# ShigemichiMatsuzaki/MSPL

Measured on AMD Instinct MI355X. Metric: images/sec pseudo-label gen, ESPDNet-UE s=2.0 480x360(->288x480) bs=16, higher is better.
Workload: dtype f32; 1 GPU; BASELINE configs[1]: ESPDNet-UE s=2.0 C=13 single-source pseudo-label gen (forward + pred+0.5aux argmax + KL uncertainty + histogram), bs=16/GPU, 16x3x288x480 fp32, hipGraph replay, 3 launches in flight per GPU, 2 consecutive batches of 16 per launch; per_gpu_batch=16, batches_in_flight=3, batches_per_launch=2, classes=13

## Files before the change

include/mspl_hip.h:

```cpp
#ifndef MSPL_HIP_H
#define MSPL_HIP_H

#include <stddef.h>
#include <stdint.h>

#ifdef __cplusplus
extern "C" {
#endif

typedef enum {
    MSPL_OK = 0,
    MSPL_ERR_BAD_SHAPE = -1,
    MSPL_ERR_UNSUPPORTED = -2,
    MSPL_ERR_NULL_POINTER = -3,
    MSPL_ERR_HIP = -4
} mspl_status;

typedef struct {
    const float* scale;
    const float* shift;
    const float* alpha;
    const float* pre_add;
    const float* residual;
    const float* reinf_r;
// ... 12 lines not shown

const char* mspl_version(void);
int mspl_abi_version(void);
size_t mspl_last_error(char* buf, size_t cap);

int mspl_eesp_dw_hff_fwd(const float* x, const float* w, const int32_t dil[4], int32_t stride,
                         int32_t N, int32_t n, int32_t H, int32_t W,
                         const mspl_epilogue_t* ep, float* out, void* stream);

int mspl_conv1x1_fwd(const float* x, const float* w, int32_t N, int32_t Cin, int32_t Cout,
                     int32_t groups, int32_t HW, const mspl_epilogue_t* ep, float* out, void* stream);

int mspl_conv3x3_fwd(const float* x, const float* w, int32_t N, int32_t Cin, int32_t Cout,
                     int32_t groups, int32_t H, int32_t W, int32_t stride, int32_t shuffle_groups,
                     const mspl_epilogue_t* ep, float* out, void* stream);

int mspl_eesp_proj_dw_hff_fits(int32_t N, int32_t Cin, int32_t n, int32_t groups, int32_t H, int32_t W, const int32_t dil[4],
                               uint32_t launch_flags);
int mspl_eesp_proj_dw_hff_fwd(const float* x, const float* wp, const float* pscale, const float* pshift, const float* palpha,
                              const float* w, const int32_t dil[4], int32_t N, int32_t Cin, int32_t n, int32_t groups,
                              int32_t H, int32_t W, const mspl_epilogue_t* ep, float* out, void* stream);

int mspl_eesp_dw_exp_fits(int32_t N, int32_t n, int32_t H, int32_t W, const int32_t dil[4], uint32_t launch_flags);
int64_t mspl_eesp_dw_exp_pack_floats(int32_t n);
int mspl_eesp_dw_exp_pack(const float* w4, const float* bscale, const float* bshift, const float* balpha, const float* wexp,
                          int32_t n, int32_t H, int32_t W, const int32_t dil[4], float* packed, void* stream);
int mspl_eesp_dw_exp_fwd(const float* r, const float* packed, const int32_t dil[4], int32_t N, int32_t n, int32_t H, int32_t W,
                         const mspl_epilogue_t* ep, float* out, void* stream);
int64_t mspl_eesp_dw_exp_next_pack_floats(int32_t n);
int mspl_eesp_dw_exp_next_pack(const float* w1, int32_t n, float* next_packed, void* stream);
int mspl_eesp_dw_exp_next_fwd(const float* r, const float* packed, const int32_t dil[4], int32_t N, int32_t n, int32_t H, int32_t W,
                              const mspl_epilogue_t* ep, float* out, const float* next_packed, const float* nscale,
                              const float* nshift, const float* nalpha, float* rnext, void* stream);

int mspl_avgpool3x3s2_fwd(const float* x, int32_t N, int32_t C, int32_t H, int32_t W,
                          const mspl_epilogue_t* ep, float* out, void* stream);

int mspl_bilinear_fwd(const float* x, int32_t N, int32_t C, int32_t Hi, int32_t Wi, int32_t Ho,
                      int32_t Wo, int32_t align_corners, const mspl_epilogue_t* ep, float* out, void* stream);

int mspl_adaptive_avgpool_fwd(const float* x, int32_t N, int32_t C, int32_t Hi, int32_t Wi,
                              int32_t Ho, int32_t Wo, const mspl_epilogue_t* ep, float* out,
                              void* stream);

int mspl_pointwise_fwd(const float* x, int32_t N, int32_t C, int32_t HW, const mspl_epilogue_t* ep,
                       float* out, void* stream);

int mspl_gap_gate_fwd(const float* x, const float* w, int32_t N, int32_t Cin, int32_t Cout,
                      int32_t HW, float* mean_ws, float* gate, void* stream);

int mspl_fusion_gate_fwd(const float* z, const float* rgb, const float* depth, int64_t count, float* out, void* stream);
int mspl_fusion_gate_bwd(const float* z, const float* rgb, const float* depth, const float* gy, int64_t count,
                         float* gz, float* grgb, float* gdepth, void* stream);

int mspl_avgpool3x3s2_psum_blocks(int32_t H, int32_t W);
int mspl_avgpool3x3s2_psum_fwd(const float* x, int32_t N, int32_t C, int32_t H, int32_t W, const mspl_epilogue_t* ep, float* out,
                               float* psum, void* stream);
int mspl_gate_from_sums_fwd(const float* psum, const float* w, int32_t N, int32_t Cin, int32_t Cout, int32_t nblk, int32_t HW,
                            float* gate, void* stream);

int64_t mspl_pyr_down_prep_lds_bytes(int32_t N, int32_t P, int32_t h, int32_t w, int32_t nb, const int32_t* hs,
                                     const int32_t* ws);
int mspl_pyr_down_prep_fwd(const float* x, int32_t N, int32_t P, int32_t h, int32_t w, int32_t nb, const int32_t* hs,
                           const int32_t* ws, const float* const* stage_w, float* const* out, void* stream);
int mspl_pyr_down_prep_train_fwd(const float* x, int32_t N, int32_t P, int32_t h, int32_t w, int32_t nb, const int32_t* hs,
                                 const int32_t* ws, const float* const* stage_w, float* const* out, float* const* pooled,
// ... 206 lines not shown
```

mspl_amd/_native.py:

```python
import ctypes
import os

import torch

_HERE = os.path.dirname(os.path.abspath(__file__))
LIB_PATH = os.environ.get('MSPL_HIP_LIB') or os.path.join(_HERE, 'lib', 'libmspl_hip.so')

c_f32p = ctypes.c_void_p
c_i32 = ctypes.c_int32
c_i64 = ctypes.c_int64


class Epilogue(ctypes.Structure):
    _fields_ = [('scale', ctypes.c_void_p), ('shift', ctypes.c_void_p), ('alpha', ctypes.c_void_p),
                ('pre_add', ctypes.c_void_p), ('residual', ctypes.c_void_p), ('reinf_r', ctypes.c_void_p),
                ('reinf_w', ctypes.c_void_p), ('gate', ctypes.c_void_p),
                ('out_ctot', c_i32), ('out_coff', c_i32), ('raw_out', ctypes.c_void_p),
                ('struct_size', ctypes.c_uint32), ('flags', ctypes.c_uint32)]


ABI_VERSION = 3
LAUNCH_THROUGHPUT = 1
LAUNCH_K2_STREAM_OFF = 2
LAUNCH_K2_STREAM_FORCE = 4


_EP = ctypes.POINTER(Epilogue)

SIGNATURES = {
    'mspl_eesp_dw_hff_fwd': [c_f32p, c_f32p, ctypes.POINTER(c_i32), c_i32, c_i32, c_i32, c_i32, c_i32, _EP,
                             c_f32p, ctypes.c_void_p],
    'mspl_eesp_proj_dw_hff_fits': [c_i32] * 6 + [ctypes.POINTER(c_i32), ctypes.c_uint32],
    'mspl_eesp_proj_dw_hff_fwd': [c_f32p] * 6 + [ctypes.POINTER(c_i32)] + [c_i32] * 6 + [_EP, c_f32p, ctypes.c_void_p],
    'mspl_eesp_dw_exp_fits': [c_i32] * 4 + [ctypes.POINTER(c_i32), ctypes.c_uint32],
    'mspl_eesp_dw_exp_pack_floats': [c_i32],
    'mspl_eesp_dw_exp_pack': [c_f32p] * 5 + [c_i32] * 3 + [ctypes.POINTER(c_i32), c_f32p, ctypes.c_void_p],
    'mspl_eesp_dw_exp_fwd': [c_f32p, c_f32p, ctypes.POINTER(c_i32)] + [c_i32] * 4 + [_EP, c_f32p, ctypes.c_void_p],
    'mspl_eesp_dw_exp_next_pack_floats': [c_i32],
    'mspl_eesp_dw_exp_next_pack': [c_f32p, c_i32, c_f32p, ctypes.c_void_p],
    'mspl_eesp_dw_exp_next_fwd': [c_f32p, c_f32p, ctypes.POINTER(c_i32)] + [c_i32] * 4 + [_EP, c_f32p] + [c_f32p] * 5 + [ctypes.c_void_p],
    'mspl_conv1x1_fwd': [c_f32p, c_f32p, c_i32, c_i32, c_i32, c_i32, c_i32, _EP, c_f32p, ctypes.c_void_p],
    'mspl_conv3x3_fwd': [c_f32p, c_f32p, c_i32, c_i32, c_i32, c_i32, c_i32, c_i32, c_i32, c_i32, _EP, c_f32p,
                         ctypes.c_void_p],
    'mspl_avgpool3x3s2_fwd': [c_f32p, c_i32, c_i32, c_i32, c_i32, _EP, c_f32p, ctypes.c_void_p],
    'mspl_bilinear_fwd': [c_f32p, c_i32, c_i32, c_i32, c_i32, c_i32, c_i32, c_i32, _EP, c_f32p, ctypes.c_void_p],
    'mspl_adaptive_avgpool_fwd': [c_f32p, c_i32, c_i32, c_i32, c_i32, c_i32, c_i32, _EP, c_f32p, ctypes.c_void_p],
    'mspl_avgpool3x3s2_psum_fwd': [c_f32p, c_i32, c_i32, c_i32, c_i32, _EP, c_f32p, c_f32p, ctypes.c_void_p],
    'mspl_avgpool3x3s2_psum_blocks': [c_i32, c_i32],
    'mspl_gate_from_sums_fwd': [c_f32p, c_f32p, c_i32, c_i32, c_i32, c_i32, c_i32, c_f32p, ctypes.c_void_p],
    'mspl_pointwise_fwd': [c_f32p, c_i32, c_i32, c_i32, _EP, c_f32p, ctypes.c_void_p],
    'mspl_gap_gate_fwd': [c_f32p, c_f32p, c_i32, c_i32, c_i32, c_i32, c_f32p, c_f32p, ctypes.c_void_p],
    'mspl_fusion_gate_fwd': [c_f32p, c_f32p, c_f32p, c_i64, c_f32p, ctypes.c_void_p],
    'mspl_fusion_gate_bwd': [c_f32p, c_f32p, c_f32p, c_f32p, c_i64, c_f32p, c_f32p, c_f32p, ctypes.c_void_p],
    'mspl_pyrpool_fused_fwd': [c_f32p, c_i32, c_i32, c_i32, c_i32, c_i32, ctypes.POINTER(c_i32), ctypes.POINTER(c_i32),
                               ctypes.POINTER(ctypes.c_void_p), ctypes.POINTER(ctypes.c_void_p), c_f32p, c_f32p, c_f32p,
                               c_f32p, _EP, c_f32p, ctypes.c_void_p],
    'mspl_pyrpool_fused_train_fwd': [c_f32p, c_i32, c_i32, c_i32, c_i32, c_i32, ctypes.POINTER(c_i32), ctypes.POINTER(c_i32),
                                     ctypes.POINTER(ctypes.c_void_p), ctypes.POINTER(ctypes.c_void_p), c_f32p, c_f32p, c_f32p,
                                     c_f32p, _EP, c_f32p, c_f32p, ctypes.c_void_p],
    'mspl_pyrpool_fused_train_fits': [c_i32] * 5 + [ctypes.POINTER(c_i32), ctypes.POINTER(c_i32)],
    'mspl_pyrpool_merge_bwd': [c_f32p] * 3 + [c_i32] * 5 + [c_f32p] * 19 + [ctypes.c_void_p],
    'mspl_pyrpool_branch_bwd_fits': [c_i32] * 5 + [ctypes.POINTER(c_i32), ctypes.POINTER(c_i32)],
    'mspl_pyrpool_branch_bwd': [c_f32p] + [c_i32] * 5 + [ctypes.POINTER(c_i32), ctypes.POINTER(c_i32)] +
                               [ctypes.POINTER(ctypes.c_void_p)] * 3 + [c_f32p, c_f32p, c_f32p, ctypes.c_void_p],
    'mspl_label_epilogue_fwd': [c_f32p, c_f32p, c_i32, c_i32, c_i32, c_i32, c_i32, c_i32, c_i32, c_i32,
                                ctypes.c_void_p, ctypes.c_void_p, c_f32p, c_f32p, c_f32p, c_f32p, ctypes.c_void_p],
    'mspl_label_epilogue_hist_fwd': [c_f32p, c_f32p, c_i32, c_i32, c_i32, c_i32, c_i32, c_i32, c_i32, c_i32,
                                     ctypes.c_void_p, ctypes.c_void_p, c_f32p, ctypes.c_void_p, c_i32, ctypes.c_void_p, c_i64,
                                     ctypes.c_void_p],
    'mspl_label_epilogue_hist_workspace_bytes': [c_i32, c_i32, c_i32],
    'mspl_label_epilogue_hist_fits': [c_i32] * 8,
    'mspl_conv_bwd_data': [c_f32p, c_f32p] + [c_i32] * 10 + [c_f32p, ctypes.c_void_p],
    'mspl_conv_bwd_weight': [c_f32p, c_f32p] + [c_i32] * 10 + [c_f32p, ctypes.c_void_p],
# ... 65 lines not shown
    'mspl_eesp_bwd_fused': [c_f32p] * 4 + [ctypes.POINTER(c_i32)] + [c_f32p] * 5 + [c_i32] * 4 + [c_f32p, ctypes.POINTER(ctypes.c_void_p)] +
                           [c_f32p] * 12 + [ctypes.c_void_p],
    'mspl_eesp_dw_bwd': [c_f32p, c_f32p, c_f32p, ctypes.POINTER(c_i32), c_i32, c_i32, c_i32, c_i32, c_i32, c_f32p,
                         ctypes.POINTER(ctypes.c_void_p), ctypes.c_void_p],
    'mspl_png_writer_create': [c_i32, c_i32],
    'mspl_png_writer_submit': [ctypes.c_void_p, ctypes.c_void_p, c_i32, c_i32, c_i32, ctypes.POINTER(ctypes.c_char_p), ctypes.c_void_p],
    'mspl_png_writer_poll': [ctypes.c_void_p, c_i64, c_i32],
    'mspl_png_writer_destroy': [ctypes.c_void_p],
    'mspl_abi_version': [],
    'mspl_sum_n': [ctypes.POINTER(ctypes.c_void_p), c_i32, c_i64, c_f32p, ctypes.c_void_p],
    'mspl_sum_n_planes': [ctypes.POINTER(ctypes.c_void_p), c_i32, c_f32p, ctypes.c_float, c_i32, c_i32, c_f32p, ctypes.c_void_p],
    'mspl_transpose_weights': [ctypes.c_void_p, ctypes.c_void_p, c_i32, ctypes.c_void_p],
    'mspl_adam_step': [c_f32p, c_f32p, c_f32p, c_f32p, c_i64] + [ctypes.c_float] * 5 + [c_i32, ctypes.c_void_p],
    'mspl_merge_labels_fwd': [ctypes.POINTER(ctypes.c_void_p), c_i32, c_i64, c_i32, c_i32, c_i32, ctypes.c_void_p,
                              ctypes.c_void_p, ctypes.c_void_p],
}


def _load():
    if not os.path.isfile(LIB_PATH):
        raise ImportError(
            'mspl_amd: %s not found. Build it with `python -c "import __graft_entry__ as g; g.build()"` or '
            '`make -C mspl_amd/csrc` (hipcc --offload-arch=gfx950). There is no CPU fallback.' % LIB_PATH)
    lib = ctypes.CDLL(LIB_PATH)
    for name, argtypes in SIGNATURES.items():
        fn = getattr(lib, name)
        fn.argtypes = argtypes
        fn.restype = ctypes.c_int
    lib.mspl_pyr_down_prep_lds_bytes.restype = ctypes.c_int64
    lib.mspl_nid_workspace_floats.restype = ctypes.c_int64
    lib.mspl_eesp_dw_exp_pack_floats.restype = ctypes.c_int64
    lib.mspl_bn_fused_workspace_bytes.restype = ctypes.c_int64
    lib.mspl_eesp_dw_exp_next_pack_floats.restype = ctypes.c_int64
    lib.mspl_label_epilogue_hist_workspace_bytes.restype = ctypes.c_int64
    lib.mspl_png_writer_create.restype = ctypes.c_void_p
    lib.mspl_png_writer_submit.restype = ctypes.c_int64
    lib.mspl_version.restype = ctypes.c_char_p
    if lib.mspl_abi_version() != ABI_VERSION:
        raise ImportError('mspl_amd: %s has ABI revision %d, this package binds revision %d: rebuild the library (make -C mspl_amd/csrc)'
                          % (LIB_PATH, lib.mspl_abi_version(), ABI_VERSION))
    lib.mspl_last_error.argtypes = [ctypes.c_char_p, ctypes.c_size_t]
    lib.mspl_last_error.restype = ctypes.c_size_t
    return lib


lib = _load()


def last_error():
    buf = ctypes.create_string_buffer(512)
    lib.mspl_last_error(buf, 512)
    return buf.value.decode()


def check(status):
    if status != 0:
        raise RuntimeError('mspl_hip (%d): %s' % (status, last_error()))


def version():
    return lib.mspl_version().decode()
```

mspl_amd/layers.py:

```python
import math
import os
import weakref

import torch
from torch import nn

from . import autograd as ag
from . import ops
from .ops import Epi

config_inp_reinf = 3
PYR_SCALES = (2.0, 1.5, 1.0, 0.5, 0.1)


_PARAM_EPOCH = [0]


def bump_param_epoch():
    _PARAM_EPOCH[0] += 1


def _key(tensors):
    return (_PARAM_EPOCH[0],) + tuple((t.data_ptr(), t._version) for t in tensors)

# ... 101 lines not shown
    cur.wait_stream(_side_stream(idx, outs[0].device, cur))
    for t in outs:
        t.record_stream(cur)


def _training_path():
    return torch.is_grad_enabled()


def _conv_train(x, conv):
    if conv.kernel_size[0] == 3 and conv.dilation[0] != 1:
        raise RuntimeError('mspl_amd: dilated 3x3 convolutions only occur inside EESP (fused branch op)')
    return ag.conv(x, conv.weight, conv.stride[0], conv.groups)


def _bn_act(z, bn, alpha=None, pre_add=None, residual=None):
    if bn.training:
        if pre_add is not None:
            z, pre_add = z + pre_add, None
        if _FUSED_BN_TRAIN:
            return ag.bn_train_prelu(z, bn, alpha, residual)
        scale, shift = ag.bn_batch_stats(z, bn)
    else:
        scale, shift = train_fold(bn)
        return ag.bn_prelu(z, bn, scale, shift, alpha, pre_add=pre_add, residual=residual)
    return ag.affine_prelu(z, scale, shift, alpha, pre_add=pre_add, residual=residual)


_FUSED_TRAIN_FWD = os.environ.get('MSPL_TRAIN_FUSED_FWD', '1') != '0'
_EESP_DW_BN = os.environ.get('MSPL_EESP_DW_BN', '1') != '0'
_CONV_SKIP = os.environ.get('MSPL_CONV_SKIP', '1') != '0'
_FUSED_BN_TRAIN = os.environ.get('MSPL_FUSED_BN_TRAIN', '1') != '0'
_FUSED_DW_EXP = os.environ.get('MSPL_EESP_EXP', '1') != '0'
_FUSED_NEXT_PROJ = os.environ.get('MSPL_EESP_NEXT', '1') != '0'
_FUSED_EESP_TRAIN = os.environ.get('MSPL_FUSED_EESP_TRAIN', '1') != '0'
_FUSED_PYR_TRAIN = os.environ.get('MSPL_FUSED_PYR_TRAIN', '1') != '0'


def _conv_bn_act(x, conv, bn, alpha=None, pre_add=None, residual=None):
    if bn.training or not _FUSED_TRAIN_FWD:
        return _bn_act(_conv_train(x, conv), bn, alpha, pre_add, residual)
    if conv.kernel_size[0] == 3 and conv.dilation[0] != 1:
        raise RuntimeError('mspl_amd: dilated 3x3 convolutions only occur inside EESP (fused branch op)')
    scale, shift = train_fold(bn)
    return ag.conv_bn_prelu(x, conv.weight, conv.stride[0], conv.groups, bn, scale, shift, alpha, pre_add, residual)


def train_fold(bn):
    def build():
        scale = bn.weight * ag.frozen_bn_inv(bn)
        return scale, torch.addcmul(bn.bias, bn.running_mean, scale, value=-1.0)
    return cached(bn, 'tfold', [bn.weight, bn.bias, bn.running_mean, bn.running_var], build)


def prefold_frozen_bn(model):
    bns = [m for m in model.modules() if isinstance(m, nn.BatchNorm2d) and not m.training]
    if not bns:
        return
    with torch.no_grad():
        invs = [ag.frozen_bn_inv(m) for m in bns]
        scales = torch._foreach_mul([m.weight for m in bns], invs)
        shifts = torch._foreach_addcmul([m.bias for m in bns], [m.running_mean for m in bns], scales, value=-1.0)
    for m, sc, sh in zip(bns, scales, shifts):
        store = m.__dict__.setdefault('_mspl_cache', {})
        store['tfold'] = (_key([m.weight, m.bias, m.running_mean, m.running_var]), (sc, sh))

# ... 128 lines not shown

class EESP(nn.Module):
    def __init__(self, nIn, nOut, stride=1, k=4, r_lim=7, down_method='esp'):
        super().__init__()
        self.stride = stride
        n = int(nOut / k)
        n1 = nOut - (k - 1) * n
        assert down_method in ['avg', 'esp'], 'One of these is suppported (avg or esp)'
        assert n == n1, "n(={}) and n1(={}) should be equal for Depth-wise Convolution ".format(n, n1)
        if k != 4:
            raise NotImplementedError('mspl_amd: the fused EESP kernel is built for k=4 branches')
        self.proj_1x1 = CBR(nIn, n, 1, stride=1, groups=k)
        self.dilations = eesp_dilations(r_lim, k)
        self.spp_dw = nn.ModuleList(CDilated(n, n, kSize=3, stride=stride, groups=n, d=d) for d in self.dilations)
        self.conv_1x1_exp = CB(nOut, nOut, 1, 1, groups=k)
        self.br_after_cat = BR(nOut)
        self.module_act = nn.PReLU(nOut)
        self.downAvg = True if down_method == 'avg' else False
        self.k = k

    def _dw_weights(self):
        ws = [m.conv.weight for m in self.spp_dw]
        return cached(self, 'w4', ws, lambda: torch.stack([w.reshape(-1, 3, 3) for w in ws]).contiguous())

    def _dw_exp_packed(self, H, W):
        br, exp = self.br_after_cat, self.conv_1x1_exp
        deps = [m.conv.weight for m in self.spp_dw] + [br.bn.weight, br.bn.bias, br.bn.running_mean, br.bn.running_var,
                                                      br.act.weight, exp.conv.weight]

        def build():
            bs, bb = bn_fold(br.bn)
            return ops.eesp_dw_exp_pack(self._dw_weights(), bs, bb, br.act.weight, exp.conv.weight, H, W, self.dilations)
        return cached(self, 'dwexp%dx%d' % (H, W), deps, build)

    def reduce_transform(self, input):
        scale, shift = bn_fold(self.br_after_cat.bn)
        pj = self.proj_1x1
        if ops.eesp_proj_dw_hff_fits(input.shape, pj.conv.out_channels, pj.conv.groups, self.dilations, self.stride):
            ps, pb = bn_fold(pj.bn)
            return ops.eesp_proj_dw_hff(input, pj.conv.weight, ps, pb, pj.act.weight, self._dw_weights(), self.dilations,
                                        pj.conv.groups, Epi(scale, shift, self.br_after_cat.act.weight))
        o1 = pj(input)
        return ops.eesp_dw_hff(o1, self._dw_weights(), self.dilations, self.stride,
                               Epi(scale, shift, self.br_after_cat.act.weight))

    def _forward_train(self, input):
        pj, br, exp = self.proj_1x1, self.br_after_cat, self.conv_1x1_exp
        if _FUSED_EESP_TRAIN and not (pj.bn.training or br.bn.training or exp.bn.training):
            def fold(bn):
                scale, shift = train_fold(bn)
                return {'scale': scale, 'shift': shift, 'mean': bn.running_mean, 'inv': ag.frozen_bn_inv(bn)}
            strided_avg = self.stride == 2 and self.downAvg
            residual = (not strided_avg) and self.stride == 1 and exp.conv.out_channels == input.shape[1]
            cfg = {'stride': self.stride, 'dil': tuple(self.dilations), 'groups': pj.conv.groups, 'residual': residual}
            ws = [m.conv.weight for m in self.spp_dw]
            return ag.EESPFn.apply(input, cfg, fold(pj.bn), fold(br.bn), fold(exp.bn), pj.conv.weight, pj.bn.weight, pj.bn.bias,
                                   pj.act.weight, ws[0], ws[1], ws[2], ws[3], br.bn.weight, br.bn.bias, br.act.weight,
                                   exp.conv.weight, exp.bn.weight, exp.bn.bias, None if strided_avg else self.module_act.weight)
        has_res = self.stride == 1 and exp.conv.out_channels == input.shape[1] and not (self.stride == 2 and self.downAvg)
        skip = input
        if has_res and pj.bn.training and _CONV_SKIP and input.requires_grad:
            z1, skip = ag.conv_skip(input, pj.conv.weight, pj.conv.groups)
            o1 = _bn_act(z1, pj.bn, pj.act.weight)
        else:
            o1 = self.proj_1x1(input)
        if br.bn.training and _EESP_DW_BN and o1.requires_grad:
# ... 105 lines not shown
                rw = (cb.conv.weight.reshape(self.nout, config_inp_reinf) * rs[:, None]).contiguous()
                shift = shift + rb
            return scale.contiguous(), shift.contiguous(), rw
        return cached(self, 'epi%d' % int(with_reinf), deps, build)

    def _forward_train(self, input, input2, alias=None):
        avg_out = ag.avgpool(input)
        eesp_out = self.eesp(input if alias is None else alias)
        reinf = None
        if input2 is not None:
            with torch.no_grad():
                pyr = input2 if isinstance(input2, ImagePyramid) else ImagePyramid(input2)
                img = pyr.at_height(avg_out.shape[2])
            if img.shape[3] != avg_out.shape[3]:
                raise RuntimeError('The size of tensor a (%d) must match the size of tensor b (%d) at non-singleton '
                                   'dimension 3' % (avg_out.shape[3], img.shape[3]))
            reinf = self.inp_reinf(img)
        return ag.down_tail(avg_out, eesp_out, self.act.weight, reinf)

    def forward(self, input, input2=None, _alias=None):
        if _training_path():
            return self._forward_train(input, input2, _alias)
        N, _, H, W = input.shape
        Ho, Wo = (H - 1) // 2 + 1, (W - 1) // 2 + 1
        out = torch.empty((N, self.nout, Ho, Wo), device=input.device, dtype=torch.float32)
        r = None
        if input2 is not None:
            pyr = input2 if isinstance(input2, ImagePyramid) else ImagePyramid(input2)
            with fork(0, (pyr.levels[0],)):
                r = self.inp_reinf[0](pyr.at_height(Ho))
            if r.shape[3] != Wo:
                raise RuntimeError('The size of tensor a (%d) must match the size of tensor b (%d) at non-singleton '
                                   'dimension 3' % (Wo, r.shape[3]))
        cat = self.eesp.reduce_transform(input)
        join(0, (r,))
        scale, shift, rw = self._epilogue_vectors(r is not None)
        ep = Epi(scale, shift, self.act.weight, reinf_r=r, reinf_w=rw)
        _, sums = ops.avgpool3x3s2(input, ep, out=(out, 0), plane_sums=True)
        _remember_plane_sums(input, sums)
        ops.conv1x1(cat, self.eesp.conv_1x1_exp.conv.weight, self.eesp.k, ep, out=(out, self.nin))
        return out


_PLANE_SUMS = weakref.WeakKeyDictionary()


class _TensorKey(object):
    __slots__ = ('__weakref__',)


def _remember_plane_sums(t, sums):
    key = getattr(t, '_mspl_key', None)
    if key is None:
        key = _TensorKey()
        t._mspl_key = key
    _PLANE_SUMS[key] = (t.data_ptr(), t._version, sums)


def _recall_plane_sums(t):
    key = getattr(t, '_mspl_key', None)
    hit = _PLANE_SUMS.get(key) if key is not None else None
    if hit is None or hit[0] != t.data_ptr() or hit[1] != t._version:
        return None
    return hit[2]


class EfficientPyrPool(nn.Module):
    def __init__(self, in_planes, proj_planes, out_planes, scales=[2.0, 1.5, 1.0, 0.5, 0.1], last_layer_br=True):
        super().__init__()
        scales = sorted(scales, reverse=True)
        self.stages = nn.ModuleList()
        self.projection_layer = DecCBR(in_planes, proj_planes, 1, 1)
        for _ in scales:
# ... 180 lines not shown
```

mspl_amd/ops.py:

```python
import ctypes

import torch

from . import _native as nat
from ._native import Epilogue, check, lib


def _stream():
    return ctypes.c_void_p(torch.cuda.current_stream().cuda_stream)


def _f32(t, name):
    if not isinstance(t, torch.Tensor) or not t.is_cuda:
        raise RuntimeError('mspl_amd: %s must be a CUDA (ROCm) tensor; there is no CPU path' % name)
    if t.dtype != torch.float32:
        raise RuntimeError('mspl_amd: %s must be float32, got %s' % (name, t.dtype))
    if not t.is_contiguous():
        t = t.contiguous()
    return t


def _p(t):
    return None if t is None else ctypes.c_void_p(t.data_ptr())

# ... 145 lines not shown
    d = (ctypes.c_int32 * 4)(*[int(v) for v in dilations])
    check(lib.mspl_eesp_dw_exp_pack(_p(w4), _p(bs), _p(bb), _p(ba), _p(wexp), n, int(H), int(W), d, _p(packed), _stream()))
    return packed


def eesp_dw_exp_next_pack(w1):
    w1 = _f32(w1, 'next projection weight')
    n = w1.shape[0]
    if w1.numel() != n * n:
        raise RuntimeError('mspl_amd: next projection weight %s, expected (%d,%d)' % (tuple(w1.shape), n, n))
    packed = torch.empty(int(lib.mspl_eesp_dw_exp_next_pack_floats(n)), device=w1.device, dtype=torch.float32)
    check(lib.mspl_eesp_dw_exp_next_pack(_p(w1), n, _p(packed), _stream()))
    return packed


def eesp_dw_exp(r, packed, dilations, ep, next_proj=None):
    r = _f32(r, 'r')
    N, n, H, W = r.shape
    packed = _vec(packed, int(lib.mspl_eesp_dw_exp_pack_floats(n)), 'packed')
    dst = torch.empty((N, 4 * n, H, W), device=r.device, dtype=torch.float32)
    s, keep = _build(ep, dst, 0, N, 4 * n, H * W)
    d = (ctypes.c_int32 * 4)(*[int(v) for v in dilations])
    if next_proj is None:
        check(lib.mspl_eesp_dw_exp_fwd(_p(r), _p(packed), d, N, n, H, W, ctypes.byref(s), _p(dst), _stream()))
        return dst
    npk = _vec(next_proj[0], int(lib.mspl_eesp_dw_exp_next_pack_floats(n)), 'next_packed')
    ns, nb, na = _vec(next_proj[1], n, 'nscale'), _vec(next_proj[2], n, 'nshift'), _vec(next_proj[3], n, 'nalpha')
    rn = torch.empty((N, n, H, W), device=r.device, dtype=torch.float32)
    check(lib.mspl_eesp_dw_exp_next_fwd(_p(r), _p(packed), d, N, n, H, W, ctypes.byref(s), _p(dst), _p(npk), _p(ns), _p(nb), _p(na), _p(rn),
                                        _stream()))
    return dst, rn


def conv1x1(x, w, groups=1, ep=None, out=None):
    x, w = _f32(x, 'x'), _f32(w, 'w')
    N, Cin, H, W = x.shape
    Cout = w.shape[0]
    if w.numel() != Cout * (Cin // groups) or Cin % groups or Cout % groups:
        raise RuntimeError('mspl_amd: conv1x1 weight %s does not match Cin=%d groups=%d' % (tuple(w.shape), Cin, groups))
    dst, coff = _dest(out, (N, Cout, H, W), x)
    s, keep = _build(ep, dst, coff, N, Cout, H * W)
    check(lib.mspl_conv1x1_fwd(_p(x), _p(w), N, Cin, Cout, groups, H * W, ctypes.byref(s), _p(dst), _stream()))
    return dst


def conv3x3(x, w, groups=1, stride=1, shuffle_groups=0, ep=None, out=None):
    x, w = _f32(x, 'x'), _f32(w, 'w')
    N, Cin, H, W = x.shape
    Cout = w.shape[0]
    if tuple(w.shape[2:]) != (3, 3) or Cin % groups or Cout % groups or w.shape[1] != Cin // groups:
        raise RuntimeError('mspl_amd: conv3x3 weight %s does not match Cin=%d groups=%d' % (tuple(w.shape), Cin, groups))
    Ho, Wo = (H - 1) // stride + 1, (W - 1) // stride + 1
    dst, coff = _dest(out, (N, Cout, Ho, Wo), x)
    s, keep = _build(ep, dst, coff, N, Cout, Ho * Wo)
    check(lib.mspl_conv3x3_fwd(_p(x), _p(w), N, Cin, Cout, groups, H, W, stride, shuffle_groups, ctypes.byref(s),
                               _p(dst), _stream()))
    return dst


def pack_dense_weight(w):
    w = _f32(w, 'w')
    Cout, Cin, kh, kw = w.shape
    return w.permute(2, 3, 0, 1).reshape(kh * kw, Cout, Cin).contiguous()


def dense_conv(x, w_packed, ksize, dilation=1, ep=None, out=None):
# ... 258 lines not shown
```

Baseline: 19640 images/s.

## Fuse strided EESP downsampler dilated depthwise, BN-PReLU and grouped 1x1 expansion into one MFMA kernel

After: 19890 images/s (median of 6 runs). +1.3%, better.

```diff
diff --git a/include/mspl_hip.h b/include/mspl_hip.h
--- a/include/mspl_hip.h
+++ b/include/mspl_hip.h
@@ -68,6 +68,13 @@
 int mspl_eesp_dw_exp_next_fwd(const float* r, const float* packed, const int32_t dil[4], int32_t N, int32_t n, int32_t H, int32_t W,
                               const mspl_epilogue_t* ep, float* out, const float* next_packed, const float* nscale,
                               const float* nshift, const float* nalpha, float* rnext, void* stream);
+
+int mspl_eesp_down_fits(int32_t N, int32_t n, int32_t H, int32_t W, const int32_t dil[4], uint32_t launch_flags);
+int64_t mspl_eesp_down_pack_floats(int32_t n);
+int mspl_eesp_down_pack(const float* w4, const float* bscale, const float* bshift, const float* balpha, const float* wexp, int32_t n,
+                        float* packed, void* stream);
+int mspl_eesp_down_fwd(const float* r, const float* packed, const int32_t dil[4], int32_t N, int32_t n, int32_t H, int32_t W,
+                       const mspl_epilogue_t* ep, float* out, void* stream);
 
 int mspl_avgpool3x3s2_fwd(const float* x, int32_t N, int32_t C, int32_t H, int32_t W,
                           const mspl_epilogue_t* ep, float* out, void* stream);
diff --git a/mspl_amd/_native.py b/mspl_amd/_native.py
--- a/mspl_amd/_native.py
+++ b/mspl_amd/_native.py
@@ -39,6 +39,10 @@
     'mspl_eesp_dw_exp_next_pack_floats': [c_i32],
     'mspl_eesp_dw_exp_next_pack': [c_f32p, c_i32, c_f32p, ctypes.c_void_p],
     'mspl_eesp_dw_exp_next_fwd': [c_f32p, c_f32p, ctypes.POINTER(c_i32)] + [c_i32] * 4 + [_EP, c_f32p] + [c_f32p] * 5 + [ctypes.c_void_p],
+    'mspl_eesp_down_fits': [c_i32] * 4 + [ctypes.POINTER(c_i32), ctypes.c_uint32],
+    'mspl_eesp_down_pack_floats': [c_i32],
+    'mspl_eesp_down_pack': [c_f32p] * 5 + [c_i32, c_f32p, ctypes.c_void_p],
+    'mspl_eesp_down_fwd': [c_f32p, c_f32p, ctypes.POINTER(c_i32)] + [c_i32] * 4 + [_EP, c_f32p, ctypes.c_void_p],
     'mspl_conv1x1_fwd': [c_f32p, c_f32p, c_i32, c_i32, c_i32, c_i32, c_i32, _EP, c_f32p, ctypes.c_void_p],
     'mspl_conv3x3_fwd': [c_f32p, c_f32p, c_i32, c_i32, c_i32, c_i32, c_i32, c_i32, c_i32, c_i32, _EP, c_f32p,
                          ctypes.c_void_p],
@@ -170,6 +174,7 @@
     lib.mspl_eesp_dw_exp_pack_floats.restype = ctypes.c_int64
     lib.mspl_bn_fused_workspace_bytes.restype = ctypes.c_int64
     lib.mspl_eesp_dw_exp_next_pack_floats.restype = ctypes.c_int64
+    lib.mspl_eesp_down_pack_floats.restype = ctypes.c_int64
     lib.mspl_label_epilogue_hist_workspace_bytes.restype = ctypes.c_int64
     lib.mspl_png_writer_create.restype = ctypes.c_void_p
     lib.mspl_png_writer_submit.restype = ctypes.c_int64
diff --git a/mspl_amd/csrc/eesp_down.hip b/mspl_amd/csrc/eesp_down.hip
--- /dev/null
+++ b/mspl_amd/csrc/eesp_down.hip
@@ -0,0 +1,315 @@
+#include "common.hpp"
+
+namespace mspl {
+
+typedef float floatx16 __attribute__((ext_vector_type(16)));
+
+template <int D0, int D1, int D2, int D3>
+struct DDil {
+    static constexpr int d(int k) { return k == 0 ? D0 : k == 1 ? D1 : k == 2 ? D2 : D3; }
+};
+
+__device__ __forceinline__ int xd_xcd_remap(int bid, int nwg) {
+    const int q = nwg >> 3, r = nwg & 7, xcd = bid & 7;
+    const int base = (xcd < r) ? xcd * (q + 1) : r * (q + 1) + (xcd - r) * q;
+    return base + (bid >> 3);
+}
+
+constexpr int XD_REC = 48;
+constexpr int XD_KC = 4;
+
+__global__ void eesp_down_pack_kernel(const float* __restrict__ w4, const float* __restrict__ bscale, const float* __restrict__ bshift,
+                                      const float* __restrict__ balpha, const float* __restrict__ wexp, int n,
+                                      float* __restrict__ dwp, float* __restrict__ ap) {
+    const int i = blockIdx.x * blockDim.x + threadIdx.x;
+    if (i < n * XD_REC) {
+        const int c = i / XD_REC, f = i - c * XD_REC;
+        const int k = f / 12, e = f - k * 12;
+        float v;
+        if (e < 9) v = w4[((size_t)k * n + c) * 9 + e];
+        else if (e == 9) v = bscale[k * n + c];
+        else if (e == 10) v = bshift[k * n + c];
+        else v = balpha[k * n + c];
+        dwp[i] = v;
+    }
+    const int nchunk = n / XD_KC, half_kc = XD_KC / 2;
+    const int total = 4 * nchunk * 64 * half_kc;
+    if (i < total) {
+        int t = i;
+        const int ii = t % half_kc;  t /= half_kc;
+        const int lane = t % 64;     t /= 64;
+        const int ch = t % nchunk;
+        const int g = t / nchunk;
+        const int m = lane & 31;
+        const int k = ch * XD_KC + 2 * ii + (lane >> 5);
+        ap[i] = m < n ? wexp[(size_t)(g * n + m) * n + k] : 0.f;
+    }
+}
+
+template <int NCH, int BW, class DS>
+__global__ __launch_bounds__(512) void eesp_down_kernel(const float* __restrict__ r, const float* __restrict__ dwp,
+                                                        const float* __restrict__ ap, const float* __restrict__ escale,
+                                                        const float* __restrict__ eshift, const float* __restrict__ ealpha,
+                                                        const float* __restrict__ reinf_r, const float* __restrict__ reinf_w,
+                                                        float* __restrict__ out, int H, int HO, int split, int ctot, int coff,
+                                                        int bands, int nwg) {
+    constexpr int MAXD = 4;
+    constexpr int TH = 2;
+    constexpr int KC = XD_KC;
+    constexpr int ROWS = 2 * (TH - 1) + 1 + 2 * MAXD;
+    constexpr int RSH = BW + 4;
+    constexpr int RS = 2 * RSH;
+    constexpr int NCHUNK = NCH / KC;
+    constexpr int ITEMS = KC * ROWS * RSH;
+    constexpr int IPT = (ITEMS + 511) / 512;
+    constexpr int AH = KC / 2;
+    static_assert(DS::d(0) <= MAXD && DS::d(1) <= MAXD && DS::d(2) <= MAXD && DS::d(3) <= MAXD, "halo of four columns / rows");
+    static_assert(BW <= 64 && (BW % 2) == 0 && NCH <= 32 && NCH % KC == 0 && NCHUNK >= 2 && KC * TH == 8, "band geometry");
+
+    constexpr int RT_F = KC * ROWS * RS, BB_F = 4 * KC * 64 * TH;
+    __shared__ __attribute__((aligned(16))) float lds_[2 * RT_F + 2 * BB_F];
+    float* const rt_[2] = {lds_, lds_ + RT_F};
+    float* const bb_[2] = {lds_ + 2 * RT_F, lds_ + 2 * RT_F + BB_F};
+
+    const int tid = threadIdx.x;
+    const int lane = tid & 63;
+    const int wave = __builtin_amdgcn_readfirstlane(tid >> 6);
+    const int li = lane & 31, half = lane >> 5;
+
+    int lid = xd_xcd_remap(blockIdx.x, nwg);
+    const int band = lid % bands;
+    const int img = lid / bands;
+    const int y0 = (band / split) * TH;
+    const int x0 = (band % split) * BW;
+    const int WI = 2 * BW * split;
+    const int WO = BW * split;
+    const int HWI = H * WI, HWO = HO * WO;
+
+    const float* rimg = r + (size_t)img * NCH * HWI;
+    float2 sv[IPT];
+    auto load_chunk = [&](int c) {
+        const float* rc = rimg + (size_t)c * KC * HWI;
+#pragma unroll
+        for (int q = 0; q < IPT; ++q) {
+            const int i = tid + 512 * q;
+            const int ic = i < ITEMS ? i : 0;
+            const int j = ic / (ROWS * RSH);
+            const int rem = ic - j * (ROWS * RSH);
+            const int row = rem / RSH, c2 = rem - row * RSH;
+            const int gy = 2 * y0 - MAXD + row, gx = 2 * x0 - 4 + 2 * c2;
+            const bool ok = gy >= 0 && gy < H && gx >= 0 && gx < WI;
+            const int go = ok ? gy * WI + gx : 0;
+            const float2 v = *reinterpret_cast<const float2*>(rc + (size_t)j * HWI + go);
+            sv[q] = ok ? v : make_float2(0.f, 0.f);
+        }
+    };
+    auto store_chunk = [&](float* dst) {
+#pragma unroll
+        for (int q = 0; q < IPT; ++q) {
+            const int i = tid + 512 * q;
+            if (i < ITEMS) {
+                const int j = i / (ROWS * RSH);
+                const int rem = i - j * (ROWS * RSH);
+                const int row = rem / RSH, c2 = rem - row * RSH;
+                float* d = dst + (j * ROWS + row) * RS + c2;
+                d[0] = sv[q].x;
+                d[RSH] = sv[q].y;
+            }
+        }
+    };
+
+    const int dj = wave & (KC - 1), dty = wave / KC;
+    const int tx = lane < BW ? lane : BW - 1;
+    const int tapbase = (2 * dty + MAXD) * RS + 2 + tx;
+    auto dw_stage = [&](int c, const float* src, float* dst) {
+        const float* rec = dwp + (size_t)(c * KC + dj) * XD_REC;
+        float wv[XD_REC];
+#pragma unroll
+        for (int i = 0; i < XD_REC; ++i) wv[i] = rec[i];
+        const float* tp = src + dj * (ROWS * RS) + tapbase;
+        const float ctr = tp[0];
+        float prev = 0.f;
+#pragma unroll
+        for (int k = 0; k < 4; ++k) {
+            const int d = DS::d(k);
+            float a = 0.f;
+#pragma unroll
+            for (int ky = 0; ky < 3; ++ky)
+#pragma unroll
+                for (int kx = 0; kx < 3; ++kx) {
+                    const int o = (kx - 1) * d;
+                    const int col = (o & 1) ? RSH + (o - 1) / 2 : o / 2;
+                    const float t = (ky == 1 && kx == 1) ? ctr : tp[(ky - 1) * d * RS + col];
+                    a = fmaf(wv[k * 12 + ky * 3 + kx], t, a);
+                }
+            a += prev;
+            prev = a;
+            float q = fmaf(a, wv[k * 12 + 9], wv[k * 12 + 10]);
+            q = q > 0.f ? q : wv[k * 12 + 11] * q;
+            dst[((k * KC + dj) * TH + dty) * 64 + lane] = q;
+        }
+    };
+
+    const int g = wave & 3, mty = wave >> 2;
+    floatx16 acc0, acc1;
+#pragma unroll
+    for (int i = 0; i < 16; ++i) { acc0[i] = 0.f; acc1[i] = 0.f; }
+    const float2* apw = reinterpret_cast<const float2*>(ap) + (size_t)g * NCHUNK * 64 + lane;
+    float2 a_cur, a_nxt;
+    auto mm_stage = [&](const float* src, const float2 av) {
+        const float* bp = src + ((g * KC + half) * TH + mty) * 64 + 2 * li;
+#pragma unroll
+        for (int i = 0; i < AH; ++i) {
+            const float2 b2 = *reinterpret_cast<const float2*>(bp + 2 * i * TH * 64);
+            const float a = i == 0 ? av.x : av.y;
+            acc0 = __builtin_amdgcn_mfma_f32_32x32x2f32(a, b2.x, acc0, 0, 0, 0);
+            acc1 = __builtin_amdgcn_mfma_f32_32x32x2f32(a, b2.y, acc1, 0, 0, 0);
+        }
+    };
+    static_assert(AH == 2, "one float2 of A per lane and chunk");
+
+    load_chunk(0);
+    a_cur = apw[0];
+    store_chunk(rt_[0]);
+    load_chunk(1);
+    __syncthreads();
+    dw_stage(0, rt_[0], bb_[0]);
+    store_chunk(rt_[1]);
+    __syncthreads();
+
+    const int yo = y0 + mty;
+    const bool pok = 2 * li < BW && yo < HO;
+    const int pix = yo * WO + x0 + 2 * li;
+    const size_t obase = ((size_t)img * ctot + coff + g * NCH + 4 * half) * HWO + (size_t)(pok ? pix : 0);
+    float2 rr[3];
+
+#pragma unroll
+    for (int c = 0; c < NCHUNK; ++c) {
+        if (c + 2 < NCHUNK) load_chunk(c + 2);
+        if (c + 1 < NCHUNK) {
+            if ((c & 1) == 0) a_nxt = apw[(c + 1) * 64]; else a_cur = apw[(c + 1) * 64];
+            dw_stage(c + 1, rt_[(c + 1) & 1], bb_[(c + 1) & 1]);
+        } else {
+#pragma unroll
+            for (int j = 0; j < 3; ++j) {
+                rr[j] = make_float2(0.f, 0.f);
+                if (reinf_r && pok) rr[j] = *reinterpret_cast<const float2*>(reinf_r + ((size_t)img * 3 + j) * HWO + pix);
+            }
+        }
+        if ((c & 1) == 0) mm_stage(bb_[c & 1], a_cur); else mm_stage(bb_[c & 1], a_nxt);
+        if (c + 2 < NCHUNK) store_chunk(rt_[c & 1]);
+        if (c + 1 < NCHUNK) __syncthreads();
+    }
+
+#pragma unroll
+    for (int rg = 0; rg < 4; ++rg) {
+        const int ml = 8 * rg + 4 * half;
+        if (ml >= NCH) continue;
+        const int cabs = coff + g * NCH + ml;
+        const float4 sc4 = *reinterpret_cast<const float4*>(escale + cabs);
+        const float4 sh4 = *reinterpret_cast<const float4*>(eshift + cabs);
+        const float4 al4 = *reinterpret_cast<const float4*>(ealpha + cabs);
+        float rw[12];
+        if (reinf_r) {
+            const float4* rwp = reinterpret_cast<const float4*>(reinf_w + (size_t)cabs * 3);
+            const float4 w0 = rwp[0], w1 = rwp[1], w2 = rwp[2];
+            rw[0] = w0.x; rw[1] = w0.y; rw[2] = w0.z; rw[3] = w0.w; rw[4] = w1.x; rw[5] = w1.y;
+            rw[6] = w1.z; rw[7] = w1.w; rw[8] = w2.x; rw[9] = w2.y; rw[10] = w2.z; rw[11] = w2.w;
+        }
+        const float scv[4] = {sc4.x, sc4.y, sc4.z, sc4.w}, shv[4] = {sh4.x, sh4.y, sh4.z, sh4.w};
+        const float alv[4] = {al4.x, al4.y, al4.z, al4.w};
+#pragma unroll
+        for (int q = 0; q < 4; ++q) {
+            const int rq = rg * 4 + q;
+            float v0 = fmaf(acc0[rq], scv[q], shv[q]);
+            float v1 = fmaf(acc1[rq], scv[q], shv[q]);
+            if (reinf_r) {
+                v0 += rw[3 * q] * rr[0].x + rw[3 * q + 1] * rr[1].x + rw[3 * q + 2] * rr[2].x;
+                v1 += rw[3 * q] * rr[0].y + rw[3 * q + 1] * rr[1].y + rw[3 * q + 2] * rr[2].y;
+            }
+            v0 = v0 > 0.f ? v0 : alv[q] * v0;
+            v1 = v1 > 0.f ? v1 : alv[q] * v1;
+            if (pok) *reinterpret_cast<float2*>(out + obase + (size_t)(q + 8 * rg) * HWO) = make_float2(v0, v1);
+        }
+    }
+}
+
+struct XdPlan {
+    int kind;
+    int BW, split;
+};
+
+static XdPlan xd_plan(int n, int H, int W, const int32_t* dil) {
+    XdPlan p = {0, 0, 0};
+    if (H < 1 || W < 2 || (W & 1)) return p;
+    if (!(dil[0] == 1 && dil[1] == 2 && dil[2] == 3 && dil[3] == 4)) return p;
+    if (n != 24 && n != 32) return p;
+    const int wo = W / 2;
+    for (int bw : {60, 64}) {
+        if (wo % bw) continue;
+        const int s = wo / bw;
+        if (s != 1 && s != 2 && s != 4) continue;
+        p.BW = bw;  p.split = s;
+        p.kind = (bw == 60 ? 1 : 3) + (n == 32 ? 1 : 0);
+        return p;
+    }
+    return p;
+}
+
+}
+
+using namespace mspl;
+
+extern "C" int mspl_eesp_down_fits(int32_t N, int32_t n, int32_t H, int32_t W, const int32_t dil[4], uint32_t flags) {
+    (void)flags;
+    if (!dil || N < 1) return 0;
+    return xd_plan(n, H, W, dil).kind != 0 ? 1 : 0;
+}
+
+extern "C" int64_t mspl_eesp_down_pack_floats(int32_t n) { return (int64_t)n * XD_REC + 4ll * (n / XD_KC) * 64 * (XD_KC / 2); }
+
+extern "C" int mspl_eesp_down_pack(const float* w4, const float* bscale, const float* bshift, const float* balpha, const float* wexp,
+                                   int32_t n, float* packed, void* stream_) {
+    MSPL_REQUIRE(w4 && bscale && bshift && balpha && wexp && packed, MSPL_ERR_NULL_POINTER, "eesp_down_pack: null pointer");
+    MSPL_REQUIRE(n == 24 || n == 32, MSPL_ERR_UNSUPPORTED, "eesp_down_pack: n=%d not covered", n);
+    const int total = (int)mspl_eesp_down_pack_floats(n);
+    hipLaunchKernelGGL(eesp_down_pack_kernel, dim3((unsigned)ceil_div(total, 256)), dim3(256), 0, static_cast<hipStream_t>(stream_), w4,
+                       bscale, bshift, balpha, wexp, n, packed, packed + (size_t)n * XD_REC);
+    MSPL_CHECK_LAUNCH("eesp_down_pack");
+    return MSPL_OK;
+}
+
+extern "C" int mspl_eesp_down_fwd(const float* r, const float* packed, const int32_t dil[4], int32_t N, int32_t n, int32_t H, int32_t W,
+                                  const mspl_epilogue_t* ep, float* out, void* stream_) {
+    MSPL_REQUIRE(r && packed && dil && ep && out, MSPL_ERR_NULL_POINTER, "eesp_down: null pointer");
+    MSPL_REQUIRE(N >= 1 && H >= 1, MSPL_ERR_BAD_SHAPE, "eesp_down: N=%d H=%d", N, H);
+    if (int rc = check_epi(ep, 4 * n, "eesp_down")) return rc;
+    MSPL_REQUIRE(ep->scale && ep->shift && ep->alpha, MSPL_ERR_NULL_POINTER, "eesp_down: the DownSampler tail needs scale, shift and alpha");
+    MSPL_REQUIRE(!ep->pre_add && !ep->residual && !ep->gate && !ep->raw_out, MSPL_ERR_UNSUPPORTED,
+                 "eesp_down: only scale/shift/alpha and the reinforcement term");
+    const XdPlan p = xd_plan(n, H, W, dil);
+    MSPL_REQUIRE(p.kind != 0, MSPL_ERR_UNSUPPORTED, "eesp_down: n=%d H=%d W=%d dil=%d,%d,%d,%d not covered", n, H, W, dil[0], dil[1], dil[2],
+                 dil[3]);
+    const int ctot = ep->out_ctot > 0 ? ep->out_ctot : 4 * n, coff = ep->out_ctot > 0 ? ep->out_coff : 0;
+    MSPL_REQUIRE((coff & 3) == 0 && (n & 7) == 0, MSPL_ERR_BAD_SHAPE, "eesp_down: channel offset %d not a multiple of 4", coff);
+    MSPL_REQUIRE((((uintptr_t)r | (uintptr_t)out | (uintptr_t)packed | (uintptr_t)ep->scale | (uintptr_t)ep->shift | (uintptr_t)ep->alpha |
+                   (uintptr_t)ep->reinf_r | (uintptr_t)ep->reinf_w) & 15) == 0, MSPL_ERR_BAD_SHAPE, "eesp_down: operands must be 16-byte aligned");
+    const int HO = (H - 1) / 2 + 1, WO = W / 2;
+    MSPL_REQUIRE((int64_t)N * n * H * W < (1ll << 31) && (int64_t)N * ctot * HO * WO < (1ll << 31), MSPL_ERR_BAD_SHAPE,
+                 "eesp_down: tensor too large");
+    const int bands = ceil_div(HO, 2) * p.split;
+    const int64_t nwg = (int64_t)N * bands;
+    MSPL_REQUIRE(nwg < (1ll << 30), MSPL_ERR_BAD_SHAPE, "eesp_down: grid too large");
+    const float* dwp = packed;
+    const float* ap = packed + (size_t)n * XD_REC;
+    hipStream_t stream = static_cast<hipStream_t>(stream_);
+#define XD_ARGS dim3((unsigned)nwg), dim3(512), 0, stream, r, dwp, ap, ep->scale, ep->shift, ep->alpha, ep->reinf_r, ep->reinf_w, out, H, HO, \
+                p.split, ctot, coff, bands, (int)nwg
+    if (p.kind == 1) hipLaunchKernelGGL((eesp_down_kernel<24, 60, DDil<1, 2, 3, 4>>), XD_ARGS);
+    else if (p.kind == 2) hipLaunchKernelGGL((eesp_down_kernel<32, 60, DDil<1, 2, 3, 4>>), XD_ARGS);
+    else if (p.kind == 3) hipLaunchKernelGGL((eesp_down_kernel<24, 64, DDil<1, 2, 3, 4>>), XD_ARGS);
+    else hipLaunchKernelGGL((eesp_down_kernel<32, 64, DDil<1, 2, 3, 4>>), XD_ARGS);
+#undef XD_ARGS
+    MSPL_CHECK_LAUNCH("eesp_down");
+    return MSPL_OK;
+}
diff --git a/mspl_amd/layers.py b/mspl_amd/layers.py
--- a/mspl_amd/layers.py
+++ b/mspl_amd/layers.py
@@ -157,6 +157,7 @@
 _CONV_SKIP = os.environ.get('MSPL_CONV_SKIP', '1') != '0'
 _FUSED_BN_TRAIN = os.environ.get('MSPL_FUSED_BN_TRAIN', '1') != '0'
 _FUSED_DW_EXP = os.environ.get('MSPL_EESP_EXP', '1') != '0'
+_FUSED_DOWN = os.environ.get('MSPL_EESP_DOWN', '1') != '0'
 _FUSED_NEXT_PROJ = os.environ.get('MSPL_EESP_NEXT', '1') != '0'
 _FUSED_EESP_TRAIN = os.environ.get('MSPL_FUSED_EESP_TRAIN', '1') != '0'
 _FUSED_PYR_TRAIN = os.environ.get('MSPL_FUSED_PYR_TRAIN', '1') != '0'
@@ -351,6 +352,16 @@
             bs, bb = bn_fold(br.bn)
             return ops.eesp_dw_exp_pack(self._dw_weights(), bs, bb, br.act.weight, exp.conv.weight, H, W, self.dilations)
         return cached(self, 'dwexp%dx%d' % (H, W), deps, build)
+
+    def _down_packed(self):
+        br, exp = self.br_after_cat, self.conv_1x1_exp
+        deps = [m.conv.weight for m in self.spp_dw] + [br.bn.weight, br.bn.bias, br.bn.running_mean, br.bn.running_var,
+                                                      br.act.weight, exp.conv.weight]
+
+        def build():
+            bs, bb = bn_fold(br.bn)
+            return ops.eesp_down_pack(self._dw_weights(), bs, bb, br.act.weight, exp.conv.weight)
+        return cached(self, 'down', deps, build)
 
     def reduce_transform(self, input):
         scale, shift = bn_fold(self.br_after_cat.bn)
@@ -522,13 +533,22 @@
             if r.shape[3] != Wo:
                 raise RuntimeError('The size of tensor a (%d) must match the size of tensor b (%d) at non-singleton '
                                    'dimension 3' % (Wo, r.shape[3]))
-        cat = self.eesp.reduce_transform(input)
+        e = self.eesp
+        pj = e.proj_1x1
+        fused = _FUSED_DOWN and e.stride == 2 and e.downAvg and ops.eesp_down_fits((N, pj.conv.out_channels, H, W), e.dilations)
+        if fused:
+            o1 = pj(input)
+        else:
+            cat = e.reduce_transform(input)
         join(0, (r,))
         scale, shift, rw = self._epilogue_vectors(r is not None)
         ep = Epi(scale, shift, self.act.weight, reinf_r=r, reinf_w=rw)
         _, sums = ops.avgpool3x3s2(input, ep, out=(out, 0), plane_sums=True)
         _remember_plane_sums(input, sums)
-        ops.conv1x1(cat, self.eesp.conv_1x1_exp.conv.weight, self.eesp.k, ep, out=(out, self.nin))
+        if fused:
+            ops.eesp_down(o1, e._down_packed(), e.dilations, ep, out=(out, self.nin))
+        else:
+            ops.conv1x1(cat, e.conv_1x1_exp.conv.weight, e.k, ep, out=(out, self.nin))
         return out
 
 
diff --git a/mspl_amd/ops.py b/mspl_amd/ops.py
--- a/mspl_amd/ops.py
+++ b/mspl_amd/ops.py
@@ -201,6 +201,35 @@
     return dst, rn
 
 
+def eesp_down_fits(shape, dilations):
+    N, n, H, W = [int(v) for v in shape]
+    d = (ctypes.c_int32 * 4)(*[int(v) for v in dilations])
+    return bool(lib.mspl_eesp_down_fits(N, n, H, W, d, current_launch_flags()))
+
+
+def eesp_down_pack(w4, bscale, bshift, balpha, wexp):
+    w4 = _f32(w4, 'w4')
+    n = w4.shape[1]
+    if tuple(w4.shape) != (4, n, 3, 3):
+        raise RuntimeError('mspl_amd: eesp_down weight %s, expected (4,%d,3,3)' % (tuple(w4.shape), n))
+    bs, bb, ba = _vec(bscale, 4 * n, 'bscale'), _vec(bshift, 4 * n, 'bshift'), _vec(balpha, 4 * n, 'balpha')
+    wexp = _vec(wexp, 4 * n * n, 'expansion weight')
+    packed = torch.empty(int(lib.mspl_eesp_down_pack_floats(n)), device=w4.device, dtype=torch.float32)
+    check(lib.mspl_eesp_down_pack(_p(w4), _p(bs), _p(bb), _p(ba), _p(wexp), n, _p(packed), _stream()))
+    return packed
+
+
+def eesp_down(r, packed, dilations, ep, out=None):
+    r = _f32(r, 'r')
+    N, n, H, W = r.shape
+    packed = _vec(packed, int(lib.mspl_eesp_down_pack_floats(n)), 'packed')
+    dst, coff = _dest(out, (N, 4 * n, (H - 1) // 2 + 1, W // 2), r)
+    s, keep = _build(ep, dst, coff, N, 4 * n, ((H - 1) // 2 + 1) * (W // 2))
+    d = (ctypes.c_int32 * 4)(*[int(v) for v in dilations])
+    check(lib.mspl_eesp_down_fwd(_p(r), _p(packed), d, N, n, H, W, ctypes.byref(s), _p(dst), _stream()))
+    return dst
+
+
 def conv1x1(x, w, groups=1, ep=None, out=None):
     x, w = _f32(x, 'x'), _f32(w, 'w')
     N, Cin, H, W = x.shape
```
